# JonasGeiping/breaching

Measured on NVIDIA H100. Metric: reconstruction iters/sec (ResNet-18 224x224, invertinggradients), higher is better.
Workload: dtype tf32

## Files before the change

### breaching_b200/csrc/engine.cu

```cuda
#include <math.h>
#include <stdlib.h>
#include <string.h>

#include <limits>
#include <string>
#include <vector>

#include "../../include/breaching_b200.h"
#include "common.cuh"
#include "igemm.cuh"
#include "layers.cuh"
#include "tokens.cuh"
#include "objective.cuh"
#include "augment.cuh"
#include "cluster_rows.cuh"

namespace bre {
void set_pdl(bool on);
static thread_local std::string g_last_error;
void set_error(const std::string& msg) { g_last_error = msg; }
static int g_pdl = -1;
bool use_pdl() {
  if (g_pdl < 0) {
    const char* e = getenv("BRE_PDL");
// ... 893 lines not shown
      return 0;
    }
    if (pC != 3) {
      BRE_LAUNCH(launch_norm_prior(input_x(), input_grad(), pn, cfg.norm_scale, cfg.norm_p, 1, sc, dpartials, dcounter, stream));
      if (cfg.orthogonality != 0)
        BRE_LAUNCH(launch_orthogonality(input_x(), input_grad(), pN, (long long)pC * pH * pW, false, sc, dpartials, dcounter, stream));
      return 0;
    }
    PriorArgs a;
    a.x = input_x(); a.grad = input_grad(); a.N = pN; a.H = pH; a.W = pW; a.accumulate = 1;
    a.tv_scale = cfg.tv_scale; a.p = cfg.tv_inner_exp; a.q = cfg.tv_outer_exp; a.eps = cfg.tv_eps;
    a.double_opponents = cfg.tv_double_opponents; a.norm_scale = cfg.norm_scale; a.norm_p = cfg.norm_p;
    BRE_LAUNCH(launch_image_priors(a, sc, dpartials, dcounter, stream));
    if (cfg.orthogonality != 0)
      BRE_LAUNCH(launch_orthogonality(input_x(), input_grad(), pN, (long long)pC * pH * pW, false, sc, dpartials, dcounter, stream));
    return 0;
  }

  int evaluate() {
    if (ms_steps > 0) return evaluate_multistep();
    if (aug_on) BRE_TRY(augment_forward());
    BRE_TRY(sweep_forward());
    BRE_TRY(sweep_backward());
    BRE_TRY(reduce_objective(cfg.objective, cfg.obj_scale, cfg.mask_value, true));
    BRE_TRY(build_chunk_modes());
    BRE_LAUNCH(launch_make_v(G, g, chunk_w, V, P_pad, cfg.objective == BRE_OBJ_MASKED_COSINE ? cfg.mask_value : -1.f, sc, stream,
                             tc_round() ? Vt : nullptr, tc_round() ? chunk_mode : nullptr));
    serialize_next_launch();
    v_settled = true;
    BRE_TRY(sweep_tangent_forward());
    BRE_TRY(deep_inversion_stats());
    BRE_TRY(sweep_tangent_backward());
    v_settled = false;
    BRE_TRY(priors());
    if (aug_on && aug_diff) BRE_TRY(augment_pull());
    return 0;
  }

  StepArgs step_args() const {
    StepArgs a;
    a.x = x; a.m = m; a.v = v; a.best = best; a.grad = gradx;
    a.grad_task = (task_grad_from_backward() && !task_grad_folded()) ? gradx_task : nullptr;
    a.lr_table = lr_table; a.n_lr = n_lr; a.lo = lo; a.hi = hi; a.n = nx; a.C = xC; a.HW = xH * xW; a.cfg = cfg;
    return a;
  }

  int label_gradient_on_device() {
    const bre_tensor_desc& lt = td(logits);
    if (seq_len > 0)
      BRE_LAUNCH(launch_token_label_grad(t[logits].val, p, t[logits].tval, lt.N, classes(), lt.C, seq_len, cfg.task_regularization, label_grad, stream));
// ... 1066 lines not shown
}

int bre_match_reduce(const float* G, const float* g, const float* chunk_weights, int64_t n, float mask_value,
                     double* sums5_host, void* stream) {
  if (!G || !g || n <= 0) { set_error("bre_match_reduce: bad arguments"); return BRE_ERR_INVALID; }
  cudaStream_t s = (cudaStream_t)stream;
  static thread_local Scalars* sc = nullptr;
  static thread_local double* partials = nullptr;
  static thread_local int* counter = nullptr;
  if (!sc) {
    BRE_TRY(dev_alloc(&sc, 1));
    BRE_TRY(dev_alloc(&partials, (long long)kMatchMaxBlocks * 5));
    BRE_TRY(dev_alloc(&counter, 1));
  }
  BRE_TRY(launch_match_reduce(G, g, chunk_weights, n, mask_value, BRE_OBJ_COSINE, 1.f, 0.f, 0.f, false, sc, partials, counter, s));
  if (sums5_host == nullptr) return BRE_OK;
  Scalars h;
  BRE_CUDA_CHECK(cudaMemcpyAsync(&h, sc, sizeof(h), cudaMemcpyDeviceToHost, s));
  BRE_CUDA_CHECK(cudaStreamSynchronize(s));
  sums5_host[0] = h.dot; sums5_host[1] = h.nG; sums5_host[2] = h.ng; sums5_host[3] = h.sq; sums5_host[4] = h.l1w;
  return BRE_OK;
}

int bre_optimizer_step(float* x, float* m, float* v, float* best, const float* grad, const float* grad_task, const float* lr_table,
                       int32_t n_lr, const float* lo, const float* hi, int64_t n, int32_t C, int32_t HW, const bre_attack_cfg* cfg,
                       float* history, int32_t max_hist, bre_step_scalars* io, void* stream) {
  if (!x || !m || !v || !best || !grad || !lr_table || !cfg || !history || !io || n <= 0 || n_lr <= 0 || C <= 0 || HW <= 0 || max_hist < 0 ||
      (cfg->boxed && (!lo || !hi)) || n % ((int64_t)C * HW) != 0) {
    set_error("bre_optimizer_step: bad arguments");
    return BRE_ERR_INVALID;
  }
  cudaStream_t s = (cudaStream_t)stream;
  Scalars h;
  memset(&h, 0, sizeof(h));
  h.match = io->match; h.task_loss = io->task_loss; h.tv = io->tv; h.norm = io->norm; h.di = io->di; h.feat = io->feat;
  h.fmin = io->fmin; h.it = io->it; h.recorded = io->recorded; h.stopped = io->stopped; h.trial = io->trial;
  Scalars* sc = nullptr; double* partials = nullptr; int* counter = nullptr;
  int rc = dev_alloc(&sc, 1);
  if (rc == 0) rc = dev_alloc(&partials, kStepMaxBlocks);
  if (rc == 0) rc = dev_alloc(&counter, 1);
  if (rc == 0 && cudaMemcpyAsync(sc, &h, sizeof(h), cudaMemcpyHostToDevice, s) != cudaSuccess) rc = BRE_ERR_CUDA;
  StepArgs a;
  a.x = x; a.m = m; a.v = v; a.best = best; a.grad = grad; a.grad_task = grad_task; a.lr_table = lr_table; a.n_lr = n_lr;
  a.lo = lo; a.hi = hi; a.n = n; a.C = C; a.HW = HW; a.cfg = *cfg;
  if (rc == 0 && cfg->grad_clip >= 0.f) rc = launch_grad_norm(a, sc, partials, counter, s);
  if (rc == 0) rc = launch_pixel_step(a, sc, s);
// ... 102 lines not shown
```

### breaching_b200/csrc/objective.cu

```cuda
#include "objective.cuh"
#include "cluster_rows.cuh"

namespace bre {

namespace {

__device__ __forceinline__ double total_objective(const Scalars* sc, float task_reg) {
  double phi = sc->match + sc->tv + sc->norm + sc->di + sc->feat;
  if (task_reg != 0.f) phi += (double)task_reg * sc->task_loss;
  return phi;
}

__device__ void finalize_objective(Scalars* sc, int objective, float scale, float tag_scale, float fudge) {
  const double dot = sc->dot, nG = sc->nG, ng = sc->ng, sq = sc->sq, l1w = sc->l1w;
  double match = 0.0, c1 = 0.0, c2 = 0.0, c3 = 0.0;
  switch (objective) {
    case BRE_OBJ_EUCLIDEAN: match = 0.5 * sq * scale; c1 = -scale; c2 = scale; break;
    case BRE_OBJ_L1: match = 0.5 * l1w * scale; c3 = 0.5 * scale; break;
    case BRE_OBJ_TAG_EUCLIDEAN: match = 0.5 * scale * (sq + tag_scale * l1w); c1 = -scale; c2 = scale; c3 = 0.5 * scale * tag_scale; break;
    case BRE_OBJ_COSINE:
    case BRE_OBJ_MASKED_COSINE:
    case BRE_OBJ_FAST_COSINE:
    case BRE_OBJ_ANGULAR: {
      const double denom = sqrt(nG) * sqrt(ng);
      const double cosv = dot / denom;
      double alpha = -1.0 / denom;
      double beta = dot / (nG * sqrt(nG) * sqrt(ng));
      if (objective == BRE_OBJ_FAST_COSINE) beta = 0.0;
      if (objective == BRE_OBJ_ANGULAR) {
        const double lo = -1.0 + fudge, hi = 1.0 - fudge;
        const double c = cosv < lo ? lo : (cosv > hi ? hi : cosv);
        match = acos(c) / 3.14159265358979323846 * scale;
        const double inside = (cosv > lo && cosv < hi) ? 1.0 : 0.0;
        const double f = inside * scale / (3.14159265358979323846 * sqrt(1.0 - c * c));
        c1 = f * alpha; c2 = f * beta;
      } else {
        match = (1.0 - cosv) * scale;
        c1 = scale * alpha; c2 = scale * beta;
      }
      break;
    }
    default: break;
  }
  sc->match = match;
  sc->c1 = (float)c1; sc->c2 = (float)c2; sc->c3 = (float)c3;
}

template <int U>
__global__ void __launch_bounds__(256) match_reduce_kernel(const float* __restrict__ G, const float* __restrict__ g,
                                                          const float* __restrict__ chunk_w, long long n, long long nchunks,
                                                          float mask_value, int objective, float scale, float tag_scale,
                                                          float fudge, bool finalize, Scalars* sc, double* partials,
                                                          int* counter) {
  pdl_prologue();
  __shared__ double scratch[32];
  __shared__ int s_last;
  double acc[5] = {0, 0, 0, 0, 0};
  const bool masked = mask_value >= 0.f;
  for (long long base = (long long)blockIdx.x * U; base < nchunks; base += (long long)gridDim.x * U) {
    float a[U][4], b[U][4];
#pragma unroll
    for (int u = 0; u < U; ++u) {
      const long long i = (base + u) * kChunk + threadIdx.x * 4;
#pragma unroll
      for (int j = 0; j < 4; ++j) { a[u][j] = 0.f; b[u][j] = 0.f; }
      if (base + u < nchunks) {
        if (i + 3 < n) {
          const float4 va = __ldg(reinterpret_cast<const float4*>(G + i));
          const float4 vb = __ldg(reinterpret_cast<const float4*>(g + i));
          a[u][0] = va.x; a[u][1] = va.y; a[u][2] = va.z; a[u][3] = va.w;
          b[u][0] = vb.x; b[u][1] = vb.y; b[u][2] = vb.z; b[u][3] = vb.w;
        } else {
          for (int j = 0; j < 4; ++j)
            if (i + j < n) { a[u][j] = G[i + j]; b[u][j] = g[i + j]; }
        }
      }
    }
#pragma unroll
    for (int u = 0; u < U; ++u) {
      const float w = (chunk_w != nullptr && base + u < nchunks) ? __ldg(chunk_w + base + u) : 1.f;
      float s0 = 0, s1 = 0, s2 = 0, s3 = 0, s4 = 0;
#pragma unroll
      for (int j = 0; j < 4; ++j) {
        float x = a[u][j], y = b[u][j];
        if (masked && !(fabsf(y) > mask_value)) { x = 0.f; y = 0.f; }
        const float df = x - y;
        s0 = fmaf(x, y, s0); s1 = fmaf(x, x, s1); s2 = fmaf(y, y, s2); s3 = fmaf(df, df, s3); s4 += fabsf(df);
      }
      acc[0] += s0; acc[1] += s1; acc[2] += s2; acc[3] += s3; acc[4] += (double)w * s4;
    }
  }
  __shared__ double wsum[5][8];
  const int lane = threadIdx.x & 31, warp = threadIdx.x >> 5;
#pragma unroll
  for (int k = 0; k < 5; ++k) {
    const double t = warp_sum(acc[k]);
    if (lane == 0) wsum[k][warp] = t;
  }
  __syncthreads();
  if (threadIdx.x < 5) {
    double t = 0.0;
#pragma unroll
    for (int w = 0; w < 8; ++w) t += wsum[threadIdx.x][w];
    partials[(long long)blockIdx.x * 5 + threadIdx.x] = t;
  }
  __threadfence();
  __syncthreads();
  if (threadIdx.x == 0) {
    const int prev = atomicAdd(counter, 1);
    s_last = (prev == (int)gridDim.x - 1);
    if (s_last) *counter = 0;
  }
  __syncthreads();
  if (!s_last) return;
  __threadfence();
#pragma unroll
  for (int k = 0; k < 5; ++k) {
    double t = 0.0;
    for (int b = threadIdx.x; b < (int)gridDim.x; b += 256) t += __ldcg(partials + (long long)b * 5 + k);
    t = warp_sum(t);
    if (lane == 0) wsum[k][warp] = t;
  }
  __syncthreads();
  if (threadIdx.x < 5) {
    double t = 0.0;
#pragma unroll
    for (int w = 0; w < 8; ++w) t += wsum[threadIdx.x][w];
    (&sc->dot)[threadIdx.x] = t;
  }
  __syncthreads();
  if (threadIdx.x == 0 && finalize) finalize_objective(sc, objective, scale, tag_scale, fudge);
}

__global__ void __launch_bounds__(256) make_v_kernel(const float* __restrict__ G, const float* __restrict__ g,
                                                    const float* __restrict__ chunk_w, float* __restrict__ v, long long n,
                                                    long long nchunks, float mask_value, const Scalars* sc, float* __restrict__ vt,
                                                    const unsigned char* __restrict__ chunk_mode) {
  pdl_prologue();
  const float c1 = sc->c1, c2 = sc->c2, c3 = sc->c3;
  const bool masked = mask_value >= 0.f;
  for (long long ch = blockIdx.x; ch < nchunks; ch += gridDim.x) {
    const long long i = ch * kChunk + threadIdx.x * 4;
    if (i >= n) continue;
    const float w3 = c3 * (chunk_w != nullptr ? __ldg(chunk_w + ch) : 1.f);
    float a[4] = {0, 0, 0, 0}, b[4] = {0, 0, 0, 0}, r[4];
    const bool full = i + 3 < n;
    if (full) {
      const float4 va = __ldg(reinterpret_cast<const float4*>(G + i));
      const float4 vb = __ldg(reinterpret_cast<const float4*>(g + i));
      a[0] = va.x; a[1] = va.y; a[2] = va.z; a[3] = va.w;
      b[0] = vb.x; b[1] = vb.y; b[2] = vb.z; b[3] = vb.w;
    } else {
      for (int j = 0; j < 4; ++j)
        if (i + j < n) { a[j] = G[i + j]; b[j] = g[i + j]; }
    }
#pragma unroll
    for (int j = 0; j < 4; ++j) {
      const float df = a[j] - b[j];
      const float sg = df > 0.f ? 1.f : (df < 0.f ? -1.f : 0.f);
      float val = fmaf(c1, b[j], fmaf(c2, a[j], w3 * sg));
      if (masked && !(fabsf(b[j]) > mask_value)) val = 0.f;
      r[j] = val;
    }
    const int mode = (vt != nullptr) ? (chunk_mode != nullptr ? (int)__ldg(chunk_mode + ch) : 2) : 0;
    if (mode != 1) {
      if (full) *reinterpret_cast<float4*>(v + i) = make_float4(r[0], r[1], r[2], r[3]);
      else
        for (int j = 0; j < 4; ++j)
          if (i + j < n) v[i + j] = r[j];
    }
    if (mode != 0) {
      if (full) *reinterpret_cast<float4*>(vt + i) = make_float4(tf32_rna(r[0]), tf32_rna(r[1]), tf32_rna(r[2]), tf32_rna(r[3]));
      else
        for (int j = 0; j < 4; ++j)
          if (i + j < n) vt[i + j] = tf32_rna(r[j]);
    }
  }
}

__device__ __forceinline__ float powx(float a, float e) {
  if (e == 1.f) return a;
  if (e == 0.f) return 1.f;
  if (e == 2.f) return a * a;
  if (e == 0.5f) return sqrtf(a);
  if (e == -0.5f) return rsqrtf(a);
  return powf(a, e);
}

struct TvD { float f, fh, fw; };
__device__ __forceinline__ TvD tv_point(float t00, float t10, float t01, float p, float q, float eps) {
  const float dh = t10 - t00, dw = t01 - t00;
  const float a = fabsf(dh) + eps, b = fabsf(dw) + eps;
  const float s = powx(a, p) + powx(b, p);
  TvD r;
  r.f = powx(s, q);
  const float common = q * powx(s, q - 1.f) * p;
  const float sh = dh > 0.f ? 1.f : (dh < 0.f ? -1.f : 0.f);
  const float sw = dw > 0.f ? 1.f : (dw < 0.f ? -1.f : 0.f);
  r.fh = common * powx(a, p - 1.f) * sh;
// ... 416 lines not shown
  __threadfence();
  double acc = 0.0;
  for (int b = threadIdx.x; b < (int)gridDim.x; b += blockDim.x) acc += partials[b];
  const double all = block_sum(acc, scratch);
  if (threadIdx.x == 0) {
    const double r = all / (double)D;
    sc->norm = overwrite ? r : sc->norm + r;
  }
}

int launch_orthogonality(const float* x, float* grad, int N, long long D, bool overwrite, Scalars* sc, double* partials, int* counter,
                         cudaStream_t s) {
  if (N < 2) return 0;
  long long blocks = (D + 255) / 256;
  const long long cap = (long long)kNumSMs * 4;
  const int grid = (int)(blocks < cap ? blocks : cap);
  BRE_KLAUNCH(orthogonality_kernel, grid, 256, 0, s, x, grad, N, D, overwrite, sc, partials, counter);
  BRE_CHECK_LAUNCH();
  return 0;
}

static int g_match_blocks_per_sm = 4, g_match_unroll = 4;

int launch_match_reduce(const float* G, const float* g, const float* chunk_w, long long n, float mask_value,
                        int objective, float scale, float tag_scale, float fudge, bool finalize, Scalars* sc,
                        double* partials, int* counter, cudaStream_t s) {
  const long long nchunks = (n + kChunk - 1) / kChunk;
  const int unroll = g_match_unroll == 8 ? 8 : 4;
  const long long groups = (nchunks + unroll - 1) / unroll;
  int cap = kNumSMs * g_match_blocks_per_sm;
  if (cap > kMatchMaxBlocks) cap = kMatchMaxBlocks;
  const int grid = (int)(groups < cap ? (groups > 0 ? groups : 1) : cap);
  if (unroll == 8)
    BRE_KLAUNCH(match_reduce_kernel<8>, grid, 256, 0, s, G, g, chunk_w, n, nchunks, mask_value, objective, scale, tag_scale, fudge,
                finalize, sc, partials, counter);
  else
    BRE_KLAUNCH(match_reduce_kernel<4>, grid, 256, 0, s, G, g, chunk_w, n, nchunks, mask_value, objective, scale, tag_scale, fudge,
                finalize, sc, partials, counter);
  BRE_CHECK_LAUNCH();
  return 0;
}

int launch_make_v(const float* G, const float* g, const float* chunk_w, float* v, long long n, float mask_value,
                  const Scalars* sc, cudaStream_t s, float* vt, const unsigned char* chunk_mode) {
  const long long nchunks = (n + kChunk - 1) / kChunk;
  const int cap = kNumSMs * 8;
  const int grid = (int)(nchunks < cap ? (nchunks > 0 ? nchunks : 1) : cap);
  BRE_KLAUNCH(make_v_kernel, grid, 256, 0, s, G, g, chunk_w, v, n, nchunks, mask_value, sc, vt, chunk_mode);
  BRE_CHECK_LAUNCH();
  return 0;
}

int launch_image_priors(const PriorArgs& a, Scalars* sc, double* partials, int* counter, cudaStream_t s) {
  dim3 grid(ceil_div(a.W, TV_TW), ceil_div(a.H, TV_TH), a.N), block(TV_TW, TV_TH);
  BRE_KLAUNCH(image_priors_kernel, grid, block, 0, s, a, sc, partials, counter);
  BRE_CHECK_LAUNCH();
  return 0;
}

int launch_norm_prior(const float* x, float* grad, long long n, float scale, float p, int accumulate, Scalars* sc, double* partials,
                      int* counter, cudaStream_t s) {
  long long b = (n + 255) / 256;
  if (b > kNumSMs * 4) b = kNumSMs * 4;
  BRE_KLAUNCH(norm_prior_kernel, (int)b, 256, 0, s, x, grad, n, scale, p, accumulate, sc, partials, counter);
  BRE_CHECK_LAUNCH();
  return 0;
}

static inline int step_grid(long long n) {
  long long b = (n + 255) / 256;
  const long long cap = kStepMaxBlocks;
  return (int)(b < cap ? (b > 0 ? b : 1) : cap);
}

int launch_grad_norm(const StepArgs& a, Scalars* sc, double* partials, int* counter, cudaStream_t s) {
// ... 54 lines not shown
```

### breaching_b200/csrc/objective.cuh

```cuda
#pragma once
#include "../../include/breaching_b200.h"
#include "common.cuh"

namespace bre {

constexpr int kChunk = 1024;

int launch_match_reduce(const float* G, const float* g, const float* chunk_w, long long n, float mask_value,
                        int objective, float scale, float tag_scale, float fudge, bool finalize, Scalars* sc,
                        double* partials, int* counter, cudaStream_t s);
constexpr int kMatchMaxBlocks = kNumSMs * 8;

int launch_make_v(const float* G, const float* g, const float* chunk_w, float* v, long long n, float mask_value,
                  const Scalars* sc, cudaStream_t s, float* vt = nullptr, const unsigned char* chunk_mode = nullptr);

struct PriorArgs {
  const float* x; float* grad; int N, H, W; int accumulate;
  float tv_scale, p, q, eps; int double_opponents;
  float norm_scale, norm_p;
};
int launch_image_priors(const PriorArgs& a, Scalars* sc, double* partials, int* counter, cudaStream_t s);
int launch_norm_prior(const float* x, float* grad, long long n, float scale, float p, int accumulate, Scalars* sc, double* partials,
                      int* counter, cudaStream_t s);
int launch_orthogonality(const float* x, float* grad, int N, long long D, bool overwrite, Scalars* sc, double* partials, int* counter,
                         cudaStream_t s);

struct StepArgs {
  float* x; float* m; float* v; float* best;
  const float* grad; const float* grad_task;
  const float* lr_table; int n_lr;
  const float* lo; const float* hi;
  long long n; int C; int HW;
  bre_attack_cfg cfg;
};
int launch_grad_norm(const StepArgs& a, Scalars* sc, double* partials, int* counter, cudaStream_t s);
int launch_pixel_step(const StepArgs& a, Scalars* sc, cudaStream_t s);
constexpr int kStepMaxBlocks = kNumSMs * 8;
// ... 14 lines not shown
```

### breaching_b200/engine.py

```python
import ctypes
import os

import torch

from . import compiler as C

_LIB = None
LIB_PATH = os.path.join(os.path.dirname(os.path.abspath(__file__)), "lib", "libbreaching_b200.so")


class EngineError(RuntimeError):
    pass


class TensorDesc(ctypes.Structure):
    _fields_ = [("N", ctypes.c_int32), ("C", ctypes.c_int32), ("H", ctypes.c_int32), ("W", ctypes.c_int32)]


class ParamDesc(ctypes.Structure):
    _fields_ = [("numel", ctypes.c_int64), ("perm", ctypes.c_int32), ("d0", ctypes.c_int32), ("d1", ctypes.c_int32),
                ("d2", ctypes.c_int32)]


class OpDesc(ctypes.Structure):
# ... 42 lines not shown
        ("objective_excludes_task", ctypes.c_int32),
    ]


OBJECTIVES = {
    "euclidean": 0, "cosine-similarity": 1, "l1": 2, "tag-euclidean": 3, "angular": 4,
    "fast-cosine-similarity": 5, "masked-cosine-similarity": 6,
}
PEARLMUTTER = {"pearlmutter-loss": "euclidean", "pearlmutter-cosine": "cosine-similarity"}
OPTIMIZERS = {
    "adam": (0, 0.9, 0.999, 1e-8, 0.0, 0.0, 0),
    "adam-safe": (0, 0.5, 0.99, 1e-4, 0.0, 0.0, 0),
    "bert-adam": (1, 0.9, 0.999, 1e-6, 0.01, 0.0, 0),
    "momgd": (2, 0.0, 0.0, 0.0, 0.0, 0.9, 1),
    "gd": (2, 0.0, 0.0, 0.0, 0.0, 0.0, 0),
}

EXPORTS = [
    "bre_engine_create", "bre_engine_destroy", "bre_engine_load_model", "bre_engine_load_targets",
    "bre_engine_load_feature_targets", "bre_engine_set_local_steps", "bre_engine_begin_trial", "bre_engine_run", "bre_engine_run_timed", "bre_engine_sync",
    "bre_engine_status", "bre_engine_read_history", "bre_engine_get_best", "bre_engine_get_candidate",
    "bre_engine_score", "bre_engine_objective_and_gradient", "bre_engine_last_terms", "bre_engine_debug_param",
    "bre_engine_debug_step_param", "bre_engine_debug_tensor", "bre_engine_debug_op", "bre_engine_launches_per_iteration", "bre_engine_set_option", "bre_match_reduce",
    "bre_total_variation", "bre_conv_gemm", "bre_last_error", "bre_version",
    "bre_engine_load_soft_labels", "bre_engine_label_gradient", "bre_engine_set_labels",
    "bre_token_layernorm", "bre_token_attention", "bre_token_match",
    "bre_engine_param_gradients", "bre_engine_bn_batch_stats", "bre_engine_forward", "bre_image_mse",
    "bre_engine_begin_joint_trial", "bre_engine_get_joint_labels", "bre_resize_bilinear",
    "bre_engine_set_augmentations", "bre_engine_last_augmentation", "bre_augment_view",
    "bre_engine_set_augmentation_stages", "bre_engine_augmentation_draws", "bre_augment_resample", "bre_augment_blur",
    "bre_engine_set_augmentations_ex", "bre_engine_set_augmentation_stages_ex", "bre_augment_view_ex", "bre_engine_augmentation_flips",
    "bre_engine_set_trial_index", "bre_engine_debug_step_state", "bre_optimizer_step", "bre_langevin_noise",
    "bre_debug_last_gemm_plan", "bre_gemm_plan", "bre_debug_row_plan", "bre_row_op",
]


def load_library(path=None):
    global _LIB
    if _LIB is not None and path is None:
        return _LIB
    path = path or LIB_PATH
    if not os.path.exists(path):
        raise EngineError(
            f"{path} not found: build it with `python -m breaching_b200.build` (there is no CPU/eager fallback)"
        )
    lib = ctypes.CDLL(path)
# ... 9 lines not shown
    lib.bre_engine_load_feature_targets.argtypes = [vp, vp, i64]
    lib.bre_engine_set_local_steps.argtypes = [vp, i32, i32, f32, vp]
    lib.bre_engine_load_soft_labels.argtypes = [vp, vp, i64]
    lib.bre_engine_label_gradient.argtypes = [vp, vp]
    lib.bre_engine_set_labels.argtypes = [vp, vp, i32]
    lib.bre_engine_begin_trial.argtypes = [vp, vp, vp, i32]
    lib.bre_engine_run.argtypes = [vp, i32]
    lib.bre_engine_sync.argtypes = [vp]
    lib.bre_engine_run_timed.argtypes = [vp, i32, P(ctypes.c_float)]
    lib.bre_engine_status.argtypes = [vp, P(i32), P(i32), P(ctypes.c_double), P(ctypes.c_double)]
    lib.bre_engine_read_history.argtypes = [vp, vp, i32]
    lib.bre_engine_get_best.argtypes = [vp, vp]
    lib.bre_engine_get_candidate.argtypes = [vp, vp]
    lib.bre_engine_score.argtypes = [vp, vp, i32, P(ctypes.c_double)]
    lib.bre_engine_objective_and_gradient.argtypes = [vp, vp, P(ctypes.c_double), vp]
    lib.bre_engine_last_terms.argtypes = [vp, P(ctypes.c_double)]
    lib.bre_engine_debug_param.argtypes = [vp, i32, i32, vp]
    lib.bre_engine_debug_step_param.argtypes = [vp, i32, i32, i32, vp]
    lib.bre_engine_debug_tensor.argtypes = [vp, i32, i32, vp]
    lib.bre_engine_debug_op.argtypes = [vp, i32, P(i32)]
    lib.bre_engine_launches_per_iteration.argtypes = [vp, P(i32)]
    lib.bre_engine_set_option.argtypes = [vp, ctypes.c_char_p, i64]
    lib.bre_match_reduce.argtypes = [vp, vp, vp, i64, f32, P(ctypes.c_double), vp]
    lib.bre_total_variation.argtypes = [vp, vp, i32, i32, i32, f32, f32, f32, f32, i32, i32, P(ctypes.c_double), vp]
    lib.bre_conv_gemm.argtypes = [i32, i32, vp, vp, vp, vp, vp] + [i32] * 9 + [vp]
    lib.bre_token_layernorm.argtypes = [i32, vp, vp, vp, vp, vp, vp, vp, vp, f32, i32, i32, vp, vp, vp, vp, i32, vp]
    lib.bre_token_attention.argtypes = [i32, vp, vp, vp, vp, i32, i32, i32, i32, vp, vp, vp, i32, vp]
    lib.bre_token_match.argtypes = [vp, vp, vp, i32, i32, i32, vp, vp]
    lib.bre_engine_begin_joint_trial.argtypes = [vp, vp, vp, i64, vp, i32]
    lib.bre_engine_get_joint_labels.argtypes = [vp, i32, vp]
    lib.bre_engine_param_gradients.argtypes = [vp, vp, vp, i32, P(vp), i32, P(ctypes.c_double)]
    lib.bre_engine_bn_batch_stats.argtypes = [vp, i32, vp, vp]
    lib.bre_engine_forward.argtypes = [vp, vp, vp]
    lib.bre_engine_set_augmentations.argtypes = [vp, i32, P(i32), P(f32), i32, f32, i32, vp, vp, i32, ctypes.c_uint64]
    lib.bre_engine_last_augmentation.argtypes = [vp, P(i32), P(i32), P(f32), P(f32)]
    lib.bre_augment_view.argtypes = [vp, vp, i32, i32, i32, i32, i32, P(i32), P(i32), P(i32), f32, i32, P(f32), P(f32), vp, vp, i32, vp, vp]
    lib.bre_engine_set_augmentation_stages.argtypes = [vp, i32, P(AugStage), i32, i32, i32, i32, i32, ctypes.c_uint64]
    lib.bre_engine_augmentation_draws.argtypes = [vp, P(i32), P(i32), P(i32), P(f32), P(f32)]
    lib.bre_augment_resample.argtypes = [vp, vp] + [i32] * 11 + [vp]
    lib.bre_engine_set_augmentations_ex.argtypes = [vp, i32, P(i32), P(f32), i32, f32, i32, i32, i32, i32, i32, vp, vp, i32, ctypes.c_uint64]
    lib.bre_engine_set_augmentation_stages_ex.argtypes = [vp, i32, P(AugStageEx), i32, i32, i32, i32, i32, ctypes.c_uint64]
    lib.bre_augment_view_ex.argtypes = [vp, vp, i32, i32, i32, i32, i32, P(i32), P(i32), P(i32), f32, i32, i32, i32, P(f32), P(f32), P(i32), P(i32),
                                        vp, vp, i32, vp, vp]
    lib.bre_engine_augmentation_flips.argtypes = [vp, P(i32), P(i32), P(i32)]
    lib.bre_augment_blur.argtypes = [vp, vp] + [i32] * 7 + [vp]
    lib.bre_resize_bilinear.argtypes = [vp, vp, i32, i32, i32, i32, i32, i32, vp]
# ... 472 lines not shown
        return dict(fused=bool(f & 1), tangent_in_unwritten=bool(f & 2), stem_columns=bool(f & 4))

    def launches_per_iteration(self):
        out = ctypes.c_int32()
        _check(self.lib, self.lib.bre_engine_launches_per_iteration(self.h, ctypes.byref(out)), "bre_engine_launches_per_iteration")
        return out.value

    def set_option(self, name, value):
        _check(self.lib, self.lib.bre_engine_set_option(self.h, name.encode(), int(value)), "bre_engine_set_option")


def match_reduce(G, g, chunk_weights=None, mask_value=-1.0, readback=True):
    lib = load_library()
    assert G.is_cuda and g.is_cuda and G.dtype == torch.float32 and G.is_contiguous() and g.is_contiguous()
    out = (ctypes.c_double * 5)()
    stream = torch.cuda.current_stream(G.device).cuda_stream
    with torch.cuda.device(G.device):
        rc = lib.bre_match_reduce(_ptr(G), _ptr(g), _ptr(chunk_weights), G.numel(), float(mask_value),
                                  out if readback else None, ctypes.c_void_p(stream))
    _check(lib, rc, "bre_match_reduce")
    return list(out) if readback else None


def optimizer_step(x, m, v, best, grad, ccfg, lr_table, history, scalars, grad_task=None, lo=None, hi=None, C=1, HW=1):
    lib = load_library()
    for t in (x, m, v, best, grad, lr_table, history, grad_task, lo, hi):
        assert t is None or (t.is_cuda and t.dtype == torch.float32 and t.is_contiguous())
    io = StepScalars()
    io.fmin = float("inf")
    for key, val in scalars.items():
        setattr(io, key, val)
    stream = torch.cuda.current_stream(x.device).cuda_stream
    with torch.cuda.device(x.device):
        rc = lib.bre_optimizer_step(_ptr(x), _ptr(m), _ptr(v), _ptr(best), _ptr(grad), _ptr(grad_task), _ptr(lr_table), lr_table.numel(),
                                    _ptr(lo), _ptr(hi), x.numel(), int(C), int(HW), ctypes.byref(ccfg), _ptr(history), history.numel(),
                                    ctypes.byref(io), ctypes.c_void_p(stream))
    _check(lib, rc, "bre_optimizer_step")
    return {name: getattr(io, name) for name, _ in StepScalars._fields_}


def langevin_noise(seed, trial, it, n, first=0, device="cuda"):
    lib = load_library()
    out = torch.empty(int(n), dtype=torch.float32, device=device)
    stream = torch.cuda.current_stream(out.device).cuda_stream
    with torch.cuda.device(out.device):
        rc = lib.bre_langevin_noise(int(seed) & 0xFFFFFFFFFFFFFFFF, int(trial), int(it), int(first), out.numel(), _ptr(out), ctypes.c_void_p(stream))
# ... 213 lines not shown
```

### include/breaching_b200.h

```cpp
#ifndef BREACHING_B200_H
#define BREACHING_B200_H

#include <stdint.h>

#ifdef __cplusplus
extern "C" {
#endif

typedef struct bre_engine bre_engine;

enum bre_status {
  BRE_OK = 0,
  BRE_ERR_INVALID = -1,
  BRE_ERR_CUDA = -2,
  BRE_ERR_STATE = -3,
  BRE_ERR_UNSUPPORTED = -4
};

enum bre_op_kind { BRE_OP_CONV = 1, BRE_OP_BNACT = 2, BRE_OP_MAXPOOL = 3, BRE_OP_AVGPOOL = 4, BRE_OP_LINEAR = 5,
                   BRE_OP_POSADD = 6,
                   BRE_OP_LAYERNORM = 7,
                   BRE_OP_ATTENTION = 8 };
enum bre_param_perm { BRE_PERM_NONE = 0, BRE_PERM_OIHW_TO_OHWI = 1, BRE_PERM_LINEAR_CHW_TO_HWC = 2 };

// ... 131 lines not shown
  bre_aug_stage stage;
  int32_t cs_mode, cs_padding, cs_fliplr, cs_flipud;
} bre_aug_stage_ex;
int bre_engine_set_augmentation_stages_ex(bre_engine* e, int32_t n_stages, const bre_aug_stage_ex* stages, int32_t N, int32_t C, int32_t H,
                                          int32_t W, int32_t differentiable, uint64_t seed);
int bre_engine_augmentation_draws(bre_engine* e, int32_t* n_stages, int32_t* o1, int32_t* o2, float* sx, float* sy);
int bre_engine_augmentation_flips(bre_engine* e, int32_t* n_stages, int32_t* fliplr, int32_t* flipud);
int bre_augment_resample(const float* x, float* out, int32_t N, int32_t C, int32_t Hi, int32_t Wi, int32_t y0, int32_t x0, int32_t wh,
                         int32_t ww, int32_t Ho, int32_t Wo, int32_t transpose, void* stream);
int bre_augment_blur(const float* x, float* out, int32_t N, int32_t C, int32_t Hi, int32_t Wi, int32_t width, int32_t stride,
                     int32_t transpose, void* stream);

int bre_engine_param_gradients(bre_engine* e, const float* data, const int64_t* labels, int32_t n_labels,
                               float* const* grads_out, int32_t n_params, double* loss_out);
int bre_engine_bn_batch_stats(bre_engine* e, int32_t bn_index, float* mean_out, float* var_out);
int bre_engine_forward(bre_engine* e, const float* data, float* logits_out);
int bre_image_mse(const float* rec, const float* ref, int32_t N, int32_t C, int32_t HW, const float* mean, const float* std,
                  int32_t clamp01, double* mse_host, void* stream);

int bre_resize_bilinear(const float* src, float* dst, int32_t N, int32_t C, int32_t Hi, int32_t Wi, int32_t Ho, int32_t Wo, void* stream);

int bre_match_reduce(const float* G, const float* g, const float* chunk_weights, int64_t n, float mask_value,
                     double* sums5_host, void* stream);
int bre_total_variation(const float* x, float* grad, int32_t N, int32_t H, int32_t W, float scale, float inner_exp,
                        float outer_exp, float eps, int32_t double_opponents, int32_t accumulate,
                        double* value_host, void* stream);
typedef struct bre_step_scalars {
  double match, task_loss, tv, norm, di, feat;
  double fmin;
  int32_t it, recorded, stopped, trial;
  double grad_norm_sq, last_objective;
} bre_step_scalars;
int bre_optimizer_step(float* x, float* m, float* v, float* best, const float* grad, const float* grad_task, const float* lr_table,
                       int32_t n_lr, const float* lo, const float* hi, int64_t n, int32_t C, int32_t HW, const bre_attack_cfg* cfg,
                       float* history, int32_t max_hist, bre_step_scalars* io, void* stream);
int bre_langevin_noise(uint64_t seed, uint32_t trial, uint32_t it, uint64_t first, int64_t n, float* out, void* stream);
int bre_token_layernorm(int32_t sweep, const float* x, const float* in1, const float* in2, const float* in3, const float* gamma,
                        const float* beta, const float* v_gamma, const float* v_beta, float eps, int32_t rows, int32_t C, float* stats,
                        float* out, float* g_gamma, float* g_beta, int32_t round_out, void* stream);
int bre_token_attention(int32_t sweep, const float* qkv, const float* in1, const float* in2, const float* in3, int32_t B, int32_t T,
                        int32_t heads, int32_t dh, float* P, float* Pd, float* out, int32_t round_out, void* stream);

int bre_token_match(const float* rec, const float* emb, const int64_t* subset, int32_t rows, int32_t d, int32_t V, int64_t* tokens,
                    void* stream);

int bre_conv_gemm(int32_t mode, int32_t backend, const float* a, const float* w, const float* a2, const float* w2,
// ... 19 lines not shown
```

Before: 715.9.

## Fuse match reduction and direction computation into one cooperative kernel

When the two gradient vectors together exceed the L2 cache size, the objective reduction and the make_v direction pass now run as a single cooperative kernel. Each block stages its first few chunks of G and g in shared memory, finishes the global reduction with a grid sync, then walks its chunks in reverse order so the second pass hits shared memory or recently cached L2 lines instead of re-reading HBM. The goal is to avoid a second full read of both gradient vectors and one kernel launch. The costs are a cooperative launch with extra shared memory and per-call host queries for device attributes and occupancy. If co-residency cannot be guaranteed, it falls back to the original two kernels.

```diff
diff --git a/breaching_b200/csrc/engine.cu b/breaching_b200/csrc/engine.cu
--- a/breaching_b200/csrc/engine.cu
+++ b/breaching_b200/csrc/engine.cu
@@ -939,10 +939,22 @@
     if (aug_on) BRE_TRY(augment_forward());
     BRE_TRY(sweep_forward());
     BRE_TRY(sweep_backward());
-    BRE_TRY(reduce_objective(cfg.objective, cfg.obj_scale, cfg.mask_value, true));
     BRE_TRY(build_chunk_modes());
-    BRE_LAUNCH(launch_make_v(G, g, chunk_w, V, P_pad, cfg.objective == BRE_OBJ_MASKED_COSINE ? cfg.mask_value : -1.f, sc, stream,
-                             tc_round() ? Vt : nullptr, tc_round() ? chunk_mode : nullptr));
+    const float mv = cfg.objective == BRE_OBJ_MASKED_COSINE ? cfg.mask_value : -1.f;
+    int dev = 0, l2 = 0;
+    BRE_CUDA_CHECK(cudaGetDevice(&dev));
+    BRE_CUDA_CHECK(cudaDeviceGetAttribute(&l2, cudaDevAttrL2CacheSize, dev));
+    int fused = 1;
+    if (2 * P_pad * (long long)sizeof(float) > l2) {
+      fused = launch_match_direction(G, g, chunk_w, V, P_pad, mv, cfg.objective, cfg.obj_scale, cfg.tag_scale, cfg.angular_fudge, sc,
+                                     dpartials, stream, tc_round() ? Vt : nullptr, tc_round() ? chunk_mode : nullptr);
+      if (fused < 0) return fused;
+      if (fused == 0) ++launch_count;
+    }
+    if (fused != 0) {
+      BRE_TRY(reduce_objective(cfg.objective, cfg.obj_scale, cfg.mask_value, true));
+      BRE_LAUNCH(launch_make_v(G, g, chunk_w, V, P_pad, mv, sc, stream, tc_round() ? Vt : nullptr, tc_round() ? chunk_mode : nullptr));
+    }
     serialize_next_launch();
     v_settled = true;
     BRE_TRY(sweep_tangent_forward());
@@ -2055,6 +2067,37 @@
   return BRE_OK;
 }
 
+int bre_match_direction(const float* G, const float* g, const float* chunk_weights, const uint8_t* chunk_mode, int64_t n, float mask_value,
+                        int32_t objective, float scale, float tag_scale, float fudge, int32_t fused, float* v, float* vt, double* out9_host,
+                        void* stream) {
+  if (!G || !g || !v || n <= 0 || (chunk_mode && !vt)) { set_error("bre_match_direction: bad arguments"); return BRE_ERR_INVALID; }
+  cudaStream_t s = (cudaStream_t)stream;
+  static thread_local Scalars* sc = nullptr;
+  static thread_local double* partials = nullptr;
+  static thread_local int* counter = nullptr;
+  if (!sc) {
+    BRE_TRY(dev_alloc(&sc, 1));
+    BRE_TRY(dev_alloc(&partials, (long long)kMatchMaxBlocks * 5));
+    BRE_TRY(dev_alloc(&counter, 1));
+  }
+  if (fused) {
+    const int rc = launch_match_direction(G, g, chunk_weights, v, n, mask_value, objective, scale, tag_scale, fudge, sc, partials, s, vt,
+                                          chunk_mode);
+    if (rc == 1) { set_error("bre_match_direction: the reduction's grid cannot be resident at once on this device"); return BRE_ERR_UNSUPPORTED; }
+    BRE_TRY(rc);
+  } else {
+    BRE_TRY(launch_match_reduce(G, g, chunk_weights, n, mask_value, objective, scale, tag_scale, fudge, true, sc, partials, counter, s));
+    BRE_TRY(launch_make_v(G, g, chunk_weights, v, n, mask_value, sc, s, vt, chunk_mode));
+  }
+  if (out9_host == nullptr) return BRE_OK;
+  Scalars h;
+  BRE_CUDA_CHECK(cudaMemcpyAsync(&h, sc, sizeof(h), cudaMemcpyDeviceToHost, s));
+  BRE_CUDA_CHECK(cudaStreamSynchronize(s));
+  const double out[9] = {h.dot, h.nG, h.ng, h.sq, h.l1w, h.match, h.c1, h.c2, h.c3};
+  memcpy(out9_host, out, sizeof(out));
+  return BRE_OK;
+}
+
 int bre_optimizer_step(float* x, float* m, float* v, float* best, const float* grad, const float* grad_task, const float* lr_table,
                        int32_t n_lr, const float* lo, const float* hi, int64_t n, int32_t C, int32_t HW, const bre_attack_cfg* cfg,
                        float* history, int32_t max_hist, bre_step_scalars* io, void* stream) {
diff --git a/breaching_b200/csrc/objective.cu b/breaching_b200/csrc/objective.cu
--- a/breaching_b200/csrc/objective.cu
+++ b/breaching_b200/csrc/objective.cu
@@ -1,3 +1,5 @@
+#include <cooperative_groups.h>
+
 #include "objective.cuh"
 #include "cluster_rows.cuh"
 
@@ -46,35 +48,47 @@
   sc->c1 = (float)c1; sc->c2 = (float)c2; sc->c3 = (float)c3;
 }
 
+__device__ __forceinline__ void load_chunk4(const float* __restrict__ G, const float* __restrict__ g, long long n, long long ch,
+                                            float a[4], float b[4]) {
+  const long long i = ch * kChunk + threadIdx.x * 4;
+#pragma unroll
+  for (int j = 0; j < 4; ++j) { a[j] = 0.f; b[j] = 0.f; }
+  if (i + 3 < n) {
+    const float4 va = __ldg(reinterpret_cast<const float4*>(G + i));
+    const float4 vb = __ldg(reinterpret_cast<const float4*>(g + i));
+    a[0] = va.x; a[1] = va.y; a[2] = va.z; a[3] = va.w;
+    b[0] = vb.x; b[1] = vb.y; b[2] = vb.z; b[3] = vb.w;
+  } else {
+    for (int j = 0; j < 4; ++j)
+      if (i + j < n) { a[j] = G[i + j]; b[j] = g[i + j]; }
+  }
+}
+
 template <int U>
-__global__ void __launch_bounds__(256) match_reduce_kernel(const float* __restrict__ G, const float* __restrict__ g,
-                                                          const float* __restrict__ chunk_w, long long n, long long nchunks,
-                                                          float mask_value, int objective, float scale, float tag_scale,
-                                                          float fudge, bool finalize, Scalars* sc, double* partials,
-                                                          int* counter) {
-  pdl_prologue();
-  __shared__ double scratch[32];
-  __shared__ int s_last;
+__device__ __forceinline__ void match_block_sums(const float* __restrict__ G, const float* __restrict__ g,
+                                                 const float* __restrict__ chunk_w, long long n, long long nchunks, float mask_value,
+                                                 double* partials, double (&wsum)[5][8], float4* stage, int nstage) {
   double acc[5] = {0, 0, 0, 0, 0};
   const bool masked = mask_value >= 0.f;
-  for (long long base = (long long)blockIdx.x * U; base < nchunks; base += (long long)gridDim.x * U) {
+  int ordinal = 0;
+  for (long long base = (long long)blockIdx.x * U; base < nchunks; base += (long long)gridDim.x * U, ordinal += U) {
     float a[U][4], b[U][4];
 #pragma unroll
     for (int u = 0; u < U; ++u) {
-      const long long i = (base + u) * kChunk + threadIdx.x * 4;
-#pragma unroll
-      for (int j = 0; j < 4; ++j) { a[u][j] = 0.f; b[u][j] = 0.f; }
       if (base + u < nchunks) {
-        if (i + 3 < n) {
-          const float4 va = __ldg(reinterpret_cast<const float4*>(G + i));
-          const float4 vb = __ldg(reinterpret_cast<const float4*>(g + i));
-          a[u][0] = va.x; a[u][1] = va.y; a[u][2] = va.z; a[u][3] = va.w;
-          b[u][0] = vb.x; b[u][1] = vb.y; b[u][2] = vb.z; b[u][3] = vb.w;
-        } else {
-          for (int j = 0; j < 4; ++j)
-            if (i + j < n) { a[u][j] = G[i + j]; b[u][j] = g[i + j]; }
+        load_chunk4(G, g, n, base + u, a[u], b[u]);
+      } else {
+#pragma unroll
+        for (int j = 0; j < 4; ++j) { a[u][j] = 0.f; b[u][j] = 0.f; }
+      }
+    }
+    if (stage != nullptr) {
+#pragma unroll
+      for (int u = 0; u < U; ++u)
+        if (ordinal + u < nstage) {
+          stage[(2 * (ordinal + u)) * 256 + threadIdx.x] = make_float4(a[u][0], a[u][1], a[u][2], a[u][3]);
+          stage[(2 * (ordinal + u) + 1) * 256 + threadIdx.x] = make_float4(b[u][0], b[u][1], b[u][2], b[u][3]);
         }
-      }
     }
 #pragma unroll
     for (int u = 0; u < U; ++u) {
@@ -90,7 +104,6 @@
       acc[0] += s0; acc[1] += s1; acc[2] += s2; acc[3] += s3; acc[4] += (double)w * s4;
     }
   }
-  __shared__ double wsum[5][8];
   const int lane = threadIdx.x & 31, warp = threadIdx.x >> 5;
 #pragma unroll
   for (int k = 0; k < 5; ++k) {
@@ -104,16 +117,10 @@
     for (int w = 0; w < 8; ++w) t += wsum[threadIdx.x][w];
     partials[(long long)blockIdx.x * 5 + threadIdx.x] = t;
   }
-  __threadfence();
-  __syncthreads();
-  if (threadIdx.x == 0) {
-    const int prev = atomicAdd(counter, 1);
-    s_last = (prev == (int)gridDim.x - 1);
-    if (s_last) *counter = 0;
-  }
-  __syncthreads();
-  if (!s_last) return;
-  __threadfence();
+}
+
+__device__ __forceinline__ void match_grid_sums(const double* partials, double (&wsum)[5][8], double* sums) {
+  const int lane = threadIdx.x & 31, warp = threadIdx.x >> 5;
 #pragma unroll
   for (int k = 0; k < 5; ++k) {
     double t = 0.0;
@@ -126,10 +133,64 @@
     double t = 0.0;
 #pragma unroll
     for (int w = 0; w < 8; ++w) t += wsum[threadIdx.x][w];
-    (&sc->dot)[threadIdx.x] = t;
-  }
-  __syncthreads();
+    sums[threadIdx.x] = t;
+  }
+  __syncthreads();
+}
+
+template <int U>
+__global__ void __launch_bounds__(256) match_reduce_kernel(const float* __restrict__ G, const float* __restrict__ g,
+                                                          const float* __restrict__ chunk_w, long long n, long long nchunks,
+                                                          float mask_value, int objective, float scale, float tag_scale,
+                                                          float fudge, bool finalize, Scalars* sc, double* partials,
+                                                          int* counter) {
+  pdl_prologue();
+  __shared__ int s_last;
+  __shared__ double wsum[5][8];
+  match_block_sums<U>(G, g, chunk_w, n, nchunks, mask_value, partials, wsum, nullptr, 0);
+  __threadfence();
+  __syncthreads();
+  if (threadIdx.x == 0) {
+    const int prev = atomicAdd(counter, 1);
+    s_last = (prev == (int)gridDim.x - 1);
+    if (s_last) *counter = 0;
+  }
+  __syncthreads();
+  if (!s_last) return;
+  __threadfence();
+  match_grid_sums(partials, wsum, &sc->dot);
   if (threadIdx.x == 0 && finalize) finalize_objective(sc, objective, scale, tag_scale, fudge);
+}
+
+__device__ __forceinline__ void direction_chunk4(const float a[4], const float b[4], long long ch, long long n, float c1, float c2,
+                                                 float c3, bool masked, float mask_value, const float* __restrict__ chunk_w,
+                                                 float* __restrict__ v, float* __restrict__ vt, const unsigned char* __restrict__ chunk_mode) {
+  const long long i = ch * kChunk + threadIdx.x * 4;
+  if (i >= n) return;
+  const float w3 = c3 * (chunk_w != nullptr ? __ldg(chunk_w + ch) : 1.f);
+  float r[4];
+  const bool full = i + 3 < n;
+#pragma unroll
+  for (int j = 0; j < 4; ++j) {
+    const float df = a[j] - b[j];
+    const float sg = df > 0.f ? 1.f : (df < 0.f ? -1.f : 0.f);
+    float val = fmaf(c1, b[j], fmaf(c2, a[j], w3 * sg));
+    if (masked && !(fabsf(b[j]) > mask_value)) val = 0.f;
+    r[j] = val;
+  }
+  const int mode = (vt != nullptr) ? (chunk_mode != nullptr ? (int)__ldg(chunk_mode + ch) : 2) : 0;
+  if (mode != 1) {
+    if (full) *reinterpret_cast<float4*>(v + i) = make_float4(r[0], r[1], r[2], r[3]);
+    else
+      for (int j = 0; j < 4; ++j)
+        if (i + j < n) v[i + j] = r[j];
+  }
+  if (mode != 0) {
+    if (full) *reinterpret_cast<float4*>(vt + i) = make_float4(tf32_rna(r[0]), tf32_rna(r[1]), tf32_rna(r[2]), tf32_rna(r[3]));
+    else
+      for (int j = 0; j < 4; ++j)
+        if (i + j < n) vt[i + j] = tf32_rna(r[j]);
+  }
 }
 
 __global__ void __launch_bounds__(256) make_v_kernel(const float* __restrict__ G, const float* __restrict__ g,
@@ -140,41 +201,56 @@
   const float c1 = sc->c1, c2 = sc->c2, c3 = sc->c3;
   const bool masked = mask_value >= 0.f;
   for (long long ch = blockIdx.x; ch < nchunks; ch += gridDim.x) {
-    const long long i = ch * kChunk + threadIdx.x * 4;
-    if (i >= n) continue;
-    const float w3 = c3 * (chunk_w != nullptr ? __ldg(chunk_w + ch) : 1.f);
-    float a[4] = {0, 0, 0, 0}, b[4] = {0, 0, 0, 0}, r[4];
-    const bool full = i + 3 < n;
-    if (full) {
-      const float4 va = __ldg(reinterpret_cast<const float4*>(G + i));
-      const float4 vb = __ldg(reinterpret_cast<const float4*>(g + i));
-      a[0] = va.x; a[1] = va.y; a[2] = va.z; a[3] = va.w;
-      b[0] = vb.x; b[1] = vb.y; b[2] = vb.z; b[3] = vb.w;
-    } else {
-      for (int j = 0; j < 4; ++j)
-        if (i + j < n) { a[j] = G[i + j]; b[j] = g[i + j]; }
-    }
-#pragma unroll
-    for (int j = 0; j < 4; ++j) {
-      const float df = a[j] - b[j];
-      const float sg = df > 0.f ? 1.f : (df < 0.f ? -1.f : 0.f);
-      float val = fmaf(c1, b[j], fmaf(c2, a[j], w3 * sg));
-      if (masked && !(fabsf(b[j]) > mask_value)) val = 0.f;
-      r[j] = val;
-    }
-    const int mode = (vt != nullptr) ? (chunk_mode != nullptr ? (int)__ldg(chunk_mode + ch) : 2) : 0;
-    if (mode != 1) {
-      if (full) *reinterpret_cast<float4*>(v + i) = make_float4(r[0], r[1], r[2], r[3]);
-      else
-        for (int j = 0; j < 4; ++j)
-          if (i + j < n) v[i + j] = r[j];
-    }
-    if (mode != 0) {
-      if (full) *reinterpret_cast<float4*>(vt + i) = make_float4(tf32_rna(r[0]), tf32_rna(r[1]), tf32_rna(r[2]), tf32_rna(r[3]));
-      else
-        for (int j = 0; j < 4; ++j)
-          if (i + j < n) vt[i + j] = tf32_rna(r[j]);
-    }
+    if (ch * kChunk + threadIdx.x * 4 >= n) continue;
+    float a[4], b[4];
+    load_chunk4(G, g, n, ch, a, b);
+    direction_chunk4(a, b, ch, n, c1, c2, c3, masked, mask_value, chunk_w, v, vt, chunk_mode);
+  }
+}
+
+template <int U>
+__global__ void __launch_bounds__(256, 4) match_direction_kernel(const float* __restrict__ G, const float* __restrict__ g,
+                                                                const float* __restrict__ chunk_w, long long n, long long nchunks,
+                                                                float mask_value, int objective, float scale, float tag_scale,
+                                                                float fudge, Scalars* sc, double* partials, float* __restrict__ v,
+                                                                float* __restrict__ vt, const unsigned char* __restrict__ chunk_mode,
+                                                                int nstage) {
+  extern __shared__ float4 stage[];
+  __shared__ double wsum[5][8];
+  __shared__ Scalars local;
+  match_block_sums<U>(G, g, chunk_w, n, nchunks, mask_value, partials, wsum, stage, nstage);
+  cooperative_groups::this_grid().sync();
+  match_grid_sums(partials, wsum, &local.dot);
+  if (threadIdx.x == 0) {
+    finalize_objective(&local, objective, scale, tag_scale, fudge);
+    if (blockIdx.x == 0) {
+      sc->dot = local.dot; sc->nG = local.nG; sc->ng = local.ng; sc->sq = local.sq; sc->l1w = local.l1w;
+      sc->match = local.match; sc->c1 = local.c1; sc->c2 = local.c2; sc->c3 = local.c3;
+    }
+  }
+  __syncthreads();
+  const float c1 = local.c1, c2 = local.c2, c3 = local.c3;
+  const bool masked = mask_value >= 0.f;
+  const long long first = (long long)blockIdx.x * U, step = (long long)gridDim.x * U;
+  if (first >= nchunks) return;
+  const long long last_base = first + (nchunks - 1 - first) / step * step;
+  int ordinal = (int)((last_base - first) / step) * U;
+  for (long long base = last_base; base >= first; base -= step, ordinal -= U) {
+    float a[U][4], b[U][4];
+#pragma unroll
+    for (int u = U - 1; u >= 0; --u) {
+      if (base + u >= nchunks) continue;
+      if (ordinal + u < nstage) {
+        const float4 sa = stage[(2 * (ordinal + u)) * 256 + threadIdx.x], sb = stage[(2 * (ordinal + u) + 1) * 256 + threadIdx.x];
+        a[u][0] = sa.x; a[u][1] = sa.y; a[u][2] = sa.z; a[u][3] = sa.w;
+        b[u][0] = sb.x; b[u][1] = sb.y; b[u][2] = sb.z; b[u][3] = sb.w;
+      } else {
+        load_chunk4(G, g, n, base + u, a[u], b[u]);
+      }
+    }
+#pragma unroll
+    for (int u = U - 1; u >= 0; --u)
+      if (base + u < nchunks) direction_chunk4(a[u], b[u], base + u, n, c1, c2, c3, masked, mask_value, chunk_w, v, vt, chunk_mode);
   }
 }
 
@@ -637,15 +713,21 @@
 
 static int g_match_blocks_per_sm = 4, g_match_unroll = 4;
 
+static int match_grid(long long n, long long* nchunks, int* unroll) {
+  *nchunks = (n + kChunk - 1) / kChunk;
+  *unroll = g_match_unroll == 8 ? 8 : 4;
+  const long long groups = (*nchunks + *unroll - 1) / *unroll;
+  int cap = kNumSMs * g_match_blocks_per_sm;
+  if (cap > kMatchMaxBlocks) cap = kMatchMaxBlocks;
+  return (int)(groups < cap ? (groups > 0 ? groups : 1) : cap);
+}
+
 int launch_match_reduce(const float* G, const float* g, const float* chunk_w, long long n, float mask_value,
                         int objective, float scale, float tag_scale, float fudge, bool finalize, Scalars* sc,
                         double* partials, int* counter, cudaStream_t s) {
-  const long long nchunks = (n + kChunk - 1) / kChunk;
-  const int unroll = g_match_unroll == 8 ? 8 : 4;
-  const long long groups = (nchunks + unroll - 1) / unroll;
-  int cap = kNumSMs * g_match_blocks_per_sm;
-  if (cap > kMatchMaxBlocks) cap = kMatchMaxBlocks;
-  const int grid = (int)(groups < cap ? (groups > 0 ? groups : 1) : cap);
+  long long nchunks;
+  int unroll;
+  const int grid = match_grid(n, &nchunks, &unroll);
   if (unroll == 8)
     BRE_KLAUNCH(match_reduce_kernel<8>, grid, 256, 0, s, G, g, chunk_w, n, nchunks, mask_value, objective, scale, tag_scale, fudge,
                 finalize, sc, partials, counter);
@@ -666,6 +748,54 @@
   return 0;
 }
 
+static int match_direction_stage(int grid, long long nchunks) {
+  int dev = 0, sms = 0, coop = 0;
+  if (cudaGetDevice(&dev) != cudaSuccess || cudaDeviceGetAttribute(&sms, cudaDevAttrMultiProcessorCount, dev) != cudaSuccess ||
+      cudaDeviceGetAttribute(&coop, cudaDevAttrCooperativeLaunch, dev) != cudaSuccess || !coop || sms <= 0)
+    return -1;
+  const long long per_block = (nchunks + grid - 1) / grid;
+  const int want = (int)(per_block < kMatchStageMax ? per_block : kMatchStageMax);
+  for (int ns = want; ns >= 0; --ns) {
+    const int bytes = ns * kMatchStageBytes;
+    if (cudaFuncSetAttribute(match_direction_kernel<4>, cudaFuncAttributeMaxDynamicSharedMemorySize, bytes) != cudaSuccess) continue;
+    int per_sm = 0;
+    if (cudaOccupancyMaxActiveBlocksPerMultiprocessor(&per_sm, match_direction_kernel<4>, 256, bytes) != cudaSuccess) continue;
+    if ((long long)per_sm * sms >= grid) return ns;
+  }
+  (void)cudaGetLastError();
+  return -1;
+}
+
+int launch_match_direction(const float* G, const float* g, const float* chunk_w, float* v, long long n, float mask_value,
+                           int objective, float scale, float tag_scale, float fudge, Scalars* sc, double* partials, cudaStream_t s,
+                           float* vt, const unsigned char* chunk_mode) {
+  long long nchunks;
+  int unroll;
+  const int grid = match_grid(n, &nchunks, &unroll);
+  if (unroll != 4) return 1;
+  const int nstage = match_direction_stage(grid, nchunks);
+  if (nstage < 0) return 1;
+  cudaLaunchConfig_t cfg;
+  memset(&cfg, 0, sizeof(cfg));
+  cfg.gridDim = dim3(grid);
+  cfg.blockDim = dim3(256);
+  cfg.dynamicSmemBytes = (size_t)nstage * kMatchStageBytes;
+  cfg.stream = s;
+  (void)consume_serialize_once();
+  cudaLaunchAttribute attr;
+  attr.id = cudaLaunchAttributeCooperative;
+  attr.val.cooperative = 1;
+  cfg.attrs = &attr;
+  cfg.numAttrs = 1;
+  const cudaError_t err = cudaLaunchKernelEx(&cfg, match_direction_kernel<4>, G, g, chunk_w, n, nchunks, mask_value, objective, scale,
+                                             tag_scale, fudge, sc, partials, v, vt, chunk_mode, nstage);
+  if (err != cudaSuccess) {
+    set_error(std::string("kernel launch failed: ") + cudaGetErrorString(err) + " at " + __FILE__ + ":" + std::to_string(__LINE__));
+    return -2;
+  }
+  return 0;
+}
+
 int launch_image_priors(const PriorArgs& a, Scalars* sc, double* partials, int* counter, cudaStream_t s) {
   dim3 grid(ceil_div(a.W, TV_TW), ceil_div(a.H, TV_TH), a.N), block(TV_TW, TV_TH);
   BRE_KLAUNCH(image_priors_kernel, grid, block, 0, s, a, sc, partials, counter);
diff --git a/breaching_b200/csrc/objective.cuh b/breaching_b200/csrc/objective.cuh
--- a/breaching_b200/csrc/objective.cuh
+++ b/breaching_b200/csrc/objective.cuh
@@ -13,6 +13,12 @@
 
 int launch_make_v(const float* G, const float* g, const float* chunk_w, float* v, long long n, float mask_value,
                   const Scalars* sc, cudaStream_t s, float* vt = nullptr, const unsigned char* chunk_mode = nullptr);
+
+int launch_match_direction(const float* G, const float* g, const float* chunk_w, float* v, long long n, float mask_value,
+                           int objective, float scale, float tag_scale, float fudge, Scalars* sc, double* partials, cudaStream_t s,
+                           float* vt = nullptr, const unsigned char* chunk_mode = nullptr);
+constexpr int kMatchStageMax = 6;
+constexpr int kMatchStageBytes = 2 * kChunk * 4;
 
 struct PriorArgs {
   const float* x; float* grad; int N, H, W; int accumulate;
diff --git a/breaching_b200/engine.py b/breaching_b200/engine.py
--- a/breaching_b200/engine.py
+++ b/breaching_b200/engine.py
@@ -88,6 +88,7 @@
     "bre_engine_status", "bre_engine_read_history", "bre_engine_get_best", "bre_engine_get_candidate",
     "bre_engine_score", "bre_engine_objective_and_gradient", "bre_engine_last_terms", "bre_engine_debug_param",
     "bre_engine_debug_step_param", "bre_engine_debug_tensor", "bre_engine_debug_op", "bre_engine_launches_per_iteration", "bre_engine_set_option", "bre_match_reduce",
+    "bre_match_direction",
     "bre_total_variation", "bre_conv_gemm", "bre_last_error", "bre_version",
     "bre_engine_load_soft_labels", "bre_engine_label_gradient", "bre_engine_set_labels",
     "bre_token_layernorm", "bre_token_attention", "bre_token_match",
@@ -143,6 +144,7 @@
     lib.bre_engine_launches_per_iteration.argtypes = [vp, P(i32)]
     lib.bre_engine_set_option.argtypes = [vp, ctypes.c_char_p, i64]
     lib.bre_match_reduce.argtypes = [vp, vp, vp, i64, f32, P(ctypes.c_double), vp]
+    lib.bre_match_direction.argtypes = [vp, vp, vp, vp, i64, f32, i32, f32, f32, f32, i32, vp, vp, P(ctypes.c_double), vp]
     lib.bre_total_variation.argtypes = [vp, vp, i32, i32, i32, f32, f32, f32, f32, i32, i32, P(ctypes.c_double), vp]
     lib.bre_conv_gemm.argtypes = [i32, i32, vp, vp, vp, vp, vp] + [i32] * 9 + [vp]
     lib.bre_token_layernorm.argtypes = [i32, vp, vp, vp, vp, vp, vp, vp, vp, f32, i32, i32, vp, vp, vp, vp, i32, vp]
@@ -661,6 +663,20 @@
     return list(out) if readback else None
 
 
+def match_direction(G, g, v, objective, scale=1.0, tag_scale=0.0, fudge=0.0, chunk_weights=None, mask_value=-1.0, vt=None,
+                    chunk_mode=None, fused=True):
+    lib = load_library()
+    assert G.is_cuda and g.is_cuda and G.dtype == torch.float32 and G.is_contiguous() and g.is_contiguous() and v.numel() == G.numel()
+    out = (ctypes.c_double * 9)()
+    stream = torch.cuda.current_stream(G.device).cuda_stream
+    with torch.cuda.device(G.device):
+        rc = lib.bre_match_direction(_ptr(G), _ptr(g), _ptr(chunk_weights), _ptr(chunk_mode), G.numel(), float(mask_value), int(objective),
+                                     float(scale), float(tag_scale), float(fudge), int(bool(fused)), _ptr(v), _ptr(vt), out,
+                                     ctypes.c_void_p(stream))
+    _check(lib, rc, "bre_match_direction")
+    return list(out)
+
+
 def optimizer_step(x, m, v, best, grad, ccfg, lr_table, history, scalars, grad_task=None, lo=None, hi=None, C=1, HW=1):
     lib = load_library()
     for t in (x, m, v, best, grad, lr_table, history, grad_task, lo, hi):
diff --git a/include/breaching_b200.h b/include/breaching_b200.h
--- a/include/breaching_b200.h
+++ b/include/breaching_b200.h
@@ -177,6 +177,9 @@
 
 int bre_match_reduce(const float* G, const float* g, const float* chunk_weights, int64_t n, float mask_value,
                      double* sums5_host, void* stream);
+int bre_match_direction(const float* G, const float* g, const float* chunk_weights, const uint8_t* chunk_mode, int64_t n, float mask_value,
+                        int32_t objective, float scale, float tag_scale, float fudge, int32_t fused, float* v, float* vt, double* out9_host,
+                        void* stream);
 int bre_total_variation(const float* x, float* grad, int32_t N, int32_t H, int32_t W, float scale, float inner_exp,
                         float outer_exp, float eps, int32_t double_opponents, int32_t accumulate,
                         double* value_host, void* stream);
```

Result: no change. 718.7 (median of 6 runs) (+0.4%).
